# dmMaze/comic-text-detector

Measured on AMD Instinct MI355X. Metric: pages/sec at 1024x1024 bs=32 (end-to-end detector, device-resident pages), higher is better.
Workload: dtype f16

## Files before the change

### comic-text-detector_amd/csrc/kernels_post.hip

```cpp
#include <algorithm>

#include "kernels.h"


namespace {

struct Cand {
  float x1, y1, x2, y2;
  float score;
  int cls;
  int idx;
  int alive;
};

__global__ void nms_filter_kernel(const float* __restrict__ blks, int B, int rows, int no, float conf_thres,
                                  Cand* __restrict__ cands, int* __restrict__ counts) {
  const long long total = (long long)B * rows;
  for (long long i = (long long)blockIdx.x * blockDim.x + threadIdx.x; i < total;
       i += (long long)gridDim.x * blockDim.x) {
    const int b = (int)(i / rows), r = (int)(i % rows);
    const float* x = blks + i * no;
    const float obj = x[4];
    if (!(obj > conf_thres)) continue;
    float best = x[5] * obj;
    int bj = 0;
    for (int j = 1; j < no - 5; ++j) {
      const float c = x[5 + j] * obj;
      if (c > best) { best = c; bj = j; }
    }
    if (!(best > conf_thres)) continue;
    const int pos = atomicAdd(&counts[b], 1);
    Cand c;
    c.x1 = x[0] - x[2] / 2;
    c.y1 = x[1] - x[3] / 2;
    c.x2 = x[0] + x[2] / 2;
    c.y2 = x[1] + x[3] / 2;
    c.score = best;
    c.cls = bj;
    c.idx = r;
    c.alive = 1;
    cands[(size_t)b * rows + pos] = c;
  }
}

struct Best { float s; int idx; int pos; };
constexpr int NMS_THREADS = 256;
constexpr int NMS_REG = 8;

__device__ __forceinline__ bool better(const Best& a, const Best& b) {
  return a.s > b.s || (a.s == b.s && a.idx < b.idx);
}

__device__ __forceinline__ Best block_argmax(Best v, Best* sh) {
  for (int off = 32; off > 0; off >>= 1) {
    Best o;
    o.s = __shfl_down(v.s, off);
    o.idx = __shfl_down(v.idx, off);
    o.pos = __shfl_down(v.pos, off);
    if (better(o, v)) v = o;
  }
  const int w = threadIdx.x >> 6, l = threadIdx.x & 63;
  __syncthreads();
  if (l == 0) sh[w] = v;
  __syncthreads();
  Best r = sh[0];
  for (int i = 1; i < (int)(blockDim.x >> 6); ++i)
    if (better(sh[i], r)) r = sh[i];
  return r;
}

__global__ __launch_bounds__(NMS_THREADS) void nms_greedy_kernel(Cand* __restrict__ cands_all, const int* __restrict__ counts,
                                                          int rows, float iou_thres, int max_det, int max_nms,
                                                          float max_wh, float* __restrict__ dets,
                                                          int* __restrict__ out_counts) {
  __shared__ Best sh[16];
  __shared__ unsigned cnt_sh;
  const int b = blockIdx.x;
  Cand* c = cands_all + (size_t)b * rows;
  const int n = counts[b];
  float* out = dets + (size_t)b * max_det * 6;

  if (n > max_nms) {
    unsigned prefix = 0;
// ... 455 lines not shown
  constexpr int LU = 4;
  for (int pb = p_begin; pb < p_end; pb += 256 * LU) {
    int root[LU], idv[LU];
#pragma unroll
    for (int u = 0; u < LU; ++u) {
      const int p = pb + 256 * u + threadIdx.x;
      root[u] = p < p_end ? labels_all[base + p] : -1;
    }
#pragma unroll
    for (int u = 0; u < LU; ++u) idv[u] = root[u] >= 0 ? ids_all[base + root[u]] : 0;
#pragma unroll
    for (int u = 0; u < LU; ++u) {
      const int p = pb + 256 * u + threadIdx.x;
      if (p < p_end && !(bg_negative && root[u] < 0)) labels_all[base + p] = idv[u];
    }
    if (!stats) continue;
#pragma unroll
    for (int u = 0; u < LU; ++u) {
      const int p0 = pb + 256 * u;
      if (p0 >= p_end) break;
      const int p = p0 + threadIdx.x;
      const bool live = p < p_end;
      const int id = idv[u];
      const int x = live ? p % W : 0, y = live ? p / W : 0;
      const int key = live ? id : -1;
      const int prev = __shfl_up(key, 1);
      const bool head = lane == 0 || prev != key || x == 0;
      const unsigned long long heads = __ballot(head);
      if (head && id > 0 && id <= max_labels) {
        const unsigned long long later = lane == 63 ? 0ull : (heads >> (lane + 1));
        const int len = later ? __ffsll((long long)later) : 64 - lane;
        int slot = -1;
        unsigned hsh = ((unsigned)id * 2654435761u) >> 25;
        for (int probe = 0; probe < 4; ++probe) {
          const int sidx = (hsh + probe) & (LB_SLOTS - 1);
          const int old = atomicCAS(&hkey[sidx], -1, id);
          if (old == -1 || old == id) {
            slot = sidx;
            break;
          }
        }
        int* s = slot >= 0 ? hst + 5 * slot : stats + ((size_t)b * max_labels + (id - 1)) * 5;
        atomicMin(s + 0, x);
        atomicMin(s + 1, y);
        atomicMax(s + 2, x + len - 1);
        atomicMax(s + 3, y);
        atomicAdd(s + 4, len);
      }
    }
  }
  if (stats) {
    __syncthreads();
    for (int sl = threadIdx.x; sl < LB_SLOTS; sl += 256) {
      const int id = hkey[sl];
      if (id <= 0) continue;
      int* s = stats + ((size_t)b * max_labels + (id - 1)) * 5;
      atomicMin(s + 0, hst[5 * sl]);
      atomicMin(s + 1, hst[5 * sl + 1]);
      atomicMax(s + 2, hst[5 * sl + 2]);
      atomicMax(s + 3, hst[5 * sl + 3]);
      atomicAdd(s + 4, hst[5 * sl + 4]);
    }
  }
}
__global__ __launch_bounds__(256) void ccl_label_kernel(int* __restrict__ labels_all, const int* __restrict__ ids_all,
                                                        int B, int H, int W, int chunks, int* __restrict__ stats,
                                                        int max_labels, int bg_negative, int nvb) {
  for (int vb = blockIdx.x; vb < nvb; vb += gridDim.x) {
    ccl_label_body(vb, labels_all, ids_all, B, H, W, chunks, stats, max_labels, bg_negative);
    __syncthreads();
  }
}

__global__ void ccl_stats_final_kernel(int* __restrict__ stats, const int* __restrict__ n_out, int max_labels) {
  const int b = blockIdx.y;
  const int n = min(n_out[b], max_labels);
  for (int l = blockIdx.x * blockDim.x + threadIdx.x; l < n; l += gridDim.x * blockDim.x) {
    int* s = stats + ((size_t)b * max_labels + l) * 5;
    s[2] = s[2] - s[0] + 1;
    s[3] = s[3] - s[1] + 1;
  }
}

__device__ __forceinline__ void ccl2_local_body(int vb, const uint8_t* __restrict__ img, int* __restrict__ parent_all,
                                                         int H, int W, int tiles_x, int tiles_y, int thresh) {
  __shared__ int lp[CT * CT];
  __shared__ unsigned mrow[2][CT];
  int bid = vb;
  const int tx = bid % tiles_x;
  bid /= tiles_x;
  const int ty = bid % tiles_y;
  const int b = bid / tiles_y;
  const size_t base = (size_t)b * H * W;
  const int x0 = tx * CT, y0 = ty * CT;
  const int lane = threadIdx.x & 63;
  const int lx = threadIdx.x & 31;
  int pix[CT * CT / 256];
#pragma unroll
  for (int k = 0; k < CT * CT / 256; ++k) {
    const int gx = x0 + lx, gy = y0 + ((threadIdx.x + 256 * k) >> 5);
    pix[k] = img[base + (gx < W && gy < H ? (size_t)gy * W + gx : (size_t)0)];
  }
#pragma unroll
  for (int k = 0; k < CT * CT / 256; ++k) {
    const int li = threadIdx.x + 256 * k;
    const int ly = li >> 5;
    const int gx = x0 + lx, gy = y0 + ly;
    const bool valid = gx < W && gy < H;
    const bool fg = valid && pix[k] > thresh;
    const unsigned long long balf = __ballot(fg), balv = __ballot(valid);
    const unsigned mf = (unsigned)(lane < 32 ? balf : balf >> 32);
    const unsigned mv = (unsigned)(lane < 32 ? balv : balv >> 32);
    const unsigned mb = mv & ~mf;
    const unsigned mine = fg ? mf : mb;
    const unsigned below = ~mine & ((1u << lx) - 1u);
    const int start = below ? 32 - __clz(below) : 0;
    lp[li] = valid ? (ly << 5) + start : -1;
    if (lx == 0) mrow[0][ly] = mf, mrow[1][ly] = mb;
  }
  __syncthreads();
#pragma unroll
  for (int k = 0; k < CT * CT / 256; ++k) {
    const int li = threadIdx.x + 256 * k;
    const int ly = li >> 5;
    if (ly == 0) continue;
    const int cls = ((mrow[0][ly] >> lx) & 1u) ? 0 : 1;
    const unsigned m = mrow[cls][ly], ma = mrow[cls][ly - 1];
    if (!((m >> lx) & 1u) || (lx > 0 && ((m >> (lx - 1)) & 1u))) continue;
    const unsigned from = m >> lx;
    const int len = (~from) ? __ffs(~from) - 1 : 32 - lx;
    unsigned run = (len >= 32 ? 0xffffffffu : ((1u << len) - 1u)) << lx;
    if (cls == 0) run |= (run << 1) | (run >> 1);
    unsigned ov = ma & run;
    while (ov) {
      const int bpos = __ffs(ov) - 1;
      const unsigned belowa = ~ma & ((1u << bpos) - 1u);
      const int sa = belowa ? 32 - __clz(belowa) : 0;
      lds_union(lp, li, ((ly - 1) << 5) + sa);
      const unsigned froma = ma >> bpos;
      const int lena = (~froma) ? __ffs(~froma) - 1 : 32 - bpos;
      ov &= ~((lena >= 32 ? 0xffffffffu : ((1u << lena) - 1u)) << bpos);
    }
  }
  __syncthreads();
#pragma unroll
  for (int k = 0; k < CT * CT / 256; ++k) {
    const int li = threadIdx.x + 256 * k;
    const int gx = x0 + lx, gy = y0 + (li >> 5);
    if (gx >= W || gy >= H) continue;
    const int r = lds_find(lp, lp[li]);
    parent_all[base + (size_t)gy * W + gx] = (y0 + (r >> 5)) * W + x0 + (r & 31);
  }
}
__global__ __launch_bounds__(256) void ccl2_local_kernel(const uint8_t* __restrict__ img, int* __restrict__ parent_all,
                                                         int H, int W, int tiles_x, int tiles_y, int thresh, int nvb) {
  for (int vb = blockIdx.x; vb < nvb; vb += gridDim.x) {
    ccl2_local_body(vb, img, parent_all, H, W, tiles_x, tiles_y, thresh);
    __syncthreads();
  }
}

__global__ __launch_bounds__(256) void ccl2_border_h_kernel(int* __restrict__ parent_all, const uint8_t* __restrict__ img_all,
                                                            int thresh, int H, int W) {
  const int x = blockIdx.x * 256 + threadIdx.x;
  const int y = CT * (blockIdx.y + 1);
  if (x >= W || y >= H) return;
  int* parent = parent_all + (size_t)blockIdx.z * H * W;
  const uint8_t* img = img_all + (size_t)blockIdx.z * H * W;
  const int p = y * W + x;
  const bool me = (int)img[p] > thresh;
  auto same = [&](int q) { return ((int)img[q] > thresh) == me; };
  const bool q = x > 0 && same(p - 1);
  const bool up = same(p - W);
  const bool ul = x > 0 && same(p - W - 1);
  if (!me) {
    if (up && !(q && ul)) uf_union(parent, p, p - W);
    return;
  }
  const bool ur = x + 1 < W && same(p - W + 1);
  if (q) {
    if (ur && !up) uf_union(parent, p, p - W + 1);
  } else if (up) {
    uf_union(parent, p, p - W);
  } else {
    if (ul) uf_union(parent, p, p - W - 1);
    if (ur) uf_union(parent, p, p - W + 1);
  }
}

__global__ __launch_bounds__(256) void ccl2_border_v_kernel(int* __restrict__ parent_all, const uint8_t* __restrict__ img_all,
                                                            int thresh, int H, int W) {
  const int y = blockIdx.x * 256 + threadIdx.x;
  const int x = CT * (blockIdx.y + 1);
  if (y >= H || x >= W) return;
  int* parent = parent_all + (size_t)blockIdx.z * H * W;
  const uint8_t* img = img_all + (size_t)blockIdx.z * H * W;
  const int p = y * W + x;
  const bool ua = y > 0, same_tile = (y % CT) != 0;
  const bool fme = (int)img[p] > thresh, fleft = (int)img[p - 1] > thresh;
  const bool fmu = ua && (int)img[p - W] > thresh, flu = ua && (int)img[p - W - 1] > thresh;
  {
    const bool me = !fme, left = !fleft, mu = ua && !fmu, lu = ua && !flu;
    if (me && left && !(same_tile && mu && lu)) uf_union(parent, p, p - 1);
  }
  {
    const bool me = fme, left = fleft, mu = fmu, lu = flu;
    if (!me && !left) return;
    if (!same_tile) {
      if (me && left) uf_union(parent, p, p - 1);
      if (me && lu) uf_union(parent, p, p - W - 1);
      if (left && mu) uf_union(parent, p - 1, p - W);
      return;
    }
    if (me && left && !(mu && lu)) uf_union(parent, p, p - 1);
    if (me && lu && !left && !mu) uf_union(parent, p, p - W - 1);
    if (left && mu && !me && !lu) uf_union(parent, p - 1, p - W);
  }
}

__device__ __forceinline__ void ccl2_flatten_count_body(int vb, int* __restrict__ parent_all, const uint8_t* __restrict__ img_all,
                                                                 int thresh, int hw, int nchunks, int* __restrict__ chunk_cnt,
                                                                 unsigned long long* __restrict__ rootmask) {
  __shared__ int sh[4];
  const int b = vb / nchunks, ch = vb % nchunks;
  int* parent = parent_all + (size_t)b * hw;
  const uint8_t* img = img_all + (size_t)b * hw;
  const int p0 = ch * RK_CHUNK + threadIdx.x;
  int lf = 0, lb = 0;
  constexpr int FU = 4;
  static_assert(RK_PER_T % FU == 0, "whole batches");
  for (int j0 = 0; j0 < RK_PER_T; j0 += FU) {
    int v[FU], g[FU], px[FU];
#pragma unroll
    for (int j = 0; j < FU; ++j) {
      const int p = p0 + 256 * (j0 + j);
      v[j] = p < hw ? uf_load(parent, p) : -1;
      px[j] = img[min(p, hw - 1)];
    }
#pragma unroll
    for (int j = 0; j < FU; ++j) g[j] = v[j] >= 0 ? uf_load(parent, v[j]) : -1;
#pragma unroll
    for (int j = 0; j < FU; ++j) {
      const int p = p0 + 256 * (j0 + j);
      bool rf = false, rb = false;
      if (v[j] >= 0) {
        const int r = g[j] == v[j] ? v[j] : uf_find(parent, g[j]);
        if (r != v[j]) parent[p] = r;
        if (r == p) {
          if (px[j] > thresh) ++lf, rf = true; else ++lb, rb = true;
        }
      }
      const unsigned long long mf = __ballot(rf), mb = __ballot(rb);
      if ((threadIdx.x & 63) == 0) {
        const size_t wi = (size_t)ch * 64 + 4 * (j0 + j) + (threadIdx.x >> 6);
        rootmask[((size_t)b * 2 + 0) * nchunks * 64 + wi] = mf;
        rootmask[((size_t)b * 2 + 1) * nchunks * 64 + wi] = mb;
      }
    }
  }
  int tf, tb;
  block_exclusive_scan(lf, sh, &tf);
  block_exclusive_scan(lb, sh, &tb);
  if (threadIdx.x == 0) {
    chunk_cnt[((size_t)b * 2 + 0) * nchunks + ch] = tf;
    chunk_cnt[((size_t)b * 2 + 1) * nchunks + ch] = tb;
  }
}
__global__ __launch_bounds__(256) void ccl2_flatten_count_kernel(int* __restrict__ parent_all, const uint8_t* __restrict__ img_all,
                                                                 int thresh, int hw, int nchunks, int* __restrict__ chunk_cnt,
                                                                 unsigned long long* __restrict__ rootmask, int nvb) {
  for (int vb = blockIdx.x; vb < nvb; vb += gridDim.x) {
    ccl2_flatten_count_body(vb, parent_all, img_all, thresh, hw, nchunks, chunk_cnt, rootmask);
    __syncthreads();
  }
}

__global__ __launch_bounds__(256) void ccl2_scan_chunks_kernel(int* __restrict__ chunk_cnt, int nchunks, int* __restrict__ n_f,
                                                               int* __restrict__ n_b) {
  __shared__ int sh[4];
  int* c = chunk_cnt + (size_t)blockIdx.x * nchunks;
  int carry = 0;
  for (int base = 0; base < nchunks; base += 256) {
    const int i = base + threadIdx.x;
    const int v = i < nchunks ? c[i] : 0;
    int total;
    const int excl = block_exclusive_scan(v, sh, &total);
    if (i < nchunks) c[i] = carry + excl;
    carry += total;
    __syncthreads();
  }
  if (threadIdx.x == 0) ((blockIdx.x & 1) ? n_b : n_f)[blockIdx.x >> 1] = carry;
}

__device__ __forceinline__ void ccl2_rank_body(int vb, const unsigned long long* __restrict__ rootmask,
                                                        int hw, int nchunks, const int* __restrict__ chunk_cnt,
                                                        int* __restrict__ ids_all, int* __restrict__ first_f,
                                                        int* __restrict__ first_b, int max_labels) {
  __shared__ int sh[2][4];
  const int b = vb / nchunks, ch = vb % nchunks;
  const int lane = threadIdx.x & 63, w = __builtin_amdgcn_readfirstlane(threadIdx.x >> 6);
  const int base = ch * RK_CHUNK + w * 1024 + lane;
  unsigned long long mf[16], mb[16];
  int cf = 0, cb = 0;
  const unsigned long long* wf = rootmask + ((size_t)b * 2 + 0) * nchunks * 64 + (size_t)ch * 64 + w * 16;
  const unsigned long long* wb = rootmask + ((size_t)b * 2 + 1) * nchunks * 64 + (size_t)ch * 64 + w * 16;
#pragma unroll
  for (int j = 0; j < 16; ++j) {
    mf[j] = wf[j];
    mb[j] = wb[j];
    cf += __popcll(mf[j]);
    cb += __popcll(mb[j]);
  }
  if (lane == 0) sh[0][w] = cf, sh[1][w] = cb;
  __syncthreads();
  int idf = chunk_cnt[((size_t)b * 2 + 0) * nchunks + ch], idb = chunk_cnt[((size_t)b * 2 + 1) * nchunks + ch];
  for (int i = 0; i < w; ++i) idf += sh[0][i], idb += sh[1][i];
  int* ids = ids_all + (size_t)b * hw;
  const unsigned long long below = lane ? (~0ull >> (64 - lane)) : 0ull;
#pragma unroll
  for (int j = 0; j < 16; ++j) {
    const int p = base + 64 * j;
    if ((mf[j] >> lane) & 1ull) {
      const int id = idf + __popcll(mf[j] & below) + 1;
      ids[p] = id;
      if (id <= max_labels) first_f[(size_t)b * max_labels + id - 1] = p;
    } else if ((mb[j] >> lane) & 1ull) {
      const int id = idb + __popcll(mb[j] & below) + 1;
      ids[p] = -id;
      if (id <= max_labels) first_b[(size_t)b * max_labels + id - 1] = p;
    }
    idf += __popcll(mf[j]);
    idb += __popcll(mb[j]);
  }
}
__global__ __launch_bounds__(256) void ccl2_rank_kernel(const unsigned long long* __restrict__ rootmask,
                                                        int hw, int nchunks, const int* __restrict__ chunk_cnt,
                                                        int* __restrict__ ids_all, int* __restrict__ first_f,
                                                        int* __restrict__ first_b, int max_labels, int nvb) {
  for (int vb = blockIdx.x; vb < nvb; vb += gridDim.x) {
    ccl2_rank_body(vb, rootmask, hw, nchunks, chunk_cnt, ids_all, first_f, first_b, max_labels);
    __syncthreads();
  }
}

__device__ __forceinline__ void ccl2_label_body(int vb, int* __restrict__ labels_all, const int* __restrict__ ids_all, int B, int H,
                                                         int W, int chunks, int* __restrict__ st_f, int* __restrict__ st_b,
                                                         int max_labels, uint8_t* __restrict__ seg_live) {
  constexpr int EMPTY = (int)0x80000000;
  __shared__ int hkey[LB_SLOTS];
  __shared__ int hst[LB_SLOTS * 5];
  const int hw = H * W;
  const int b = vb / chunks, ch = vb % chunks;
  const int p_begin = ch * LB_CHUNK, p_end = min(hw, p_begin + LB_CHUNK);
  const size_t base = (size_t)b * hw;
  for (int s = threadIdx.x; s < LB_SLOTS; s += 256) {
    hkey[s] = EMPTY;
    hst[5 * s] = W, hst[5 * s + 1] = H, hst[5 * s + 2] = -1, hst[5 * s + 3] = -1, hst[5 * s + 4] = 0;
  }
  __syncthreads();
  const int lane = threadIdx.x & 63;
  auto row_of = [&](int id) { return (id > 0 ? st_f : st_b) + ((size_t)b * max_labels + ((id > 0 ? id : -id) - 1)) * 5; };
  constexpr int LU = 4;
  for (int pb = p_begin; pb < p_end; pb += 256 * LU) {
    int root[LU], idv[LU];
#pragma unroll
    for (int u = 0; u < LU; ++u) {
      const int p = pb + 256 * u + threadIdx.x;
      root[u] = p < p_end ? labels_all[base + p] : -1;
    }
#pragma unroll
    for (int u = 0; u < LU; ++u) idv[u] = root[u] >= 0 ? ids_all[base + root[u]] : 0;
#pragma unroll
    for (int u = 0; u < LU; ++u) {
      const int p = pb + 256 * u + threadIdx.x;
      if (p < p_end) labels_all[base + p] = idv[u];
    }
#pragma unroll
    for (int u = 0; u < LU; ++u) {
      const int p0 = pb + 256 * u;
      if (p0 >= p_end) break;
      const int p = p0 + threadIdx.x;
      const bool live = p < p_end;
      const int id = idv[u];
      const int x = live ? p % W : 0, y = live ? p / W : 0;
      if (seg_live) {
        const unsigned long long other = __ballot(live && id != -1);
        const int q0 = p0 + ((int)threadIdx.x & ~63);
        if (lane == 0 && q0 < p_end) seg_live[(size_t)b * ((hw + 63) >> 6) + (q0 >> 6)] = other ? 1 : 0;
      }
      const int prev = __shfl_up(id, 1);
      const bool head = lane == 0 || prev != id || x == 0;
      const unsigned long long heads = __ballot(head);
      const int mag = id > 0 ? id : -id;
      if (head && id != 0 && mag <= max_labels) {
        const unsigned long long later = lane == 63 ? 0ull : (heads >> (lane + 1));
        const int len = later ? __ffsll((long long)later) : 64 - lane;
        int slot = -1;
        const unsigned hsh = ((unsigned)id * 2654435761u) >> 25;
        for (int probe = 0; probe < 4; ++probe) {
          const int sidx = (hsh + probe) & (LB_SLOTS - 1);
          const int old = atomicCAS(&hkey[sidx], EMPTY, id);
          if (old == EMPTY || old == id) {
            slot = sidx;
            break;
          }
        }
        int* s = slot >= 0 ? hst + 5 * slot : row_of(id);
        atomicMin(s + 0, x);
        atomicMin(s + 1, y);
        atomicMax(s + 2, x + len - 1);
        atomicMax(s + 3, y);
        atomicAdd(s + 4, len);
      }
    }
  }
  __syncthreads();
  for (int sl = threadIdx.x; sl < LB_SLOTS; sl += 256) {
    const int id = hkey[sl];
    if (id == EMPTY) continue;
    int* s = row_of(id);
    atomicMin(s + 0, hst[5 * sl]);
    atomicMin(s + 1, hst[5 * sl + 1]);
    atomicMax(s + 2, hst[5 * sl + 2]);
    atomicMax(s + 3, hst[5 * sl + 3]);
    atomicAdd(s + 4, hst[5 * sl + 4]);
  }
}
__global__ __launch_bounds__(256) void ccl2_label_kernel(int* __restrict__ labels_all, const int* __restrict__ ids_all, int B, int H,
                                                         int W, int chunks, int* __restrict__ st_f, int* __restrict__ st_b,
                                                         int max_labels, int nvb, uint8_t* __restrict__ seg_live) {
  for (int vb = blockIdx.x; vb < nvb; vb += gridDim.x) {
    ccl2_label_body(vb, labels_all, ids_all, B, H, W, chunks, st_f, st_b, max_labels, seg_live);
    __syncthreads();
  }
}


inline int capped(int nvb) { return std::max(1, std::min(nvb, g_tail_max_blocks)); }

inline int grid_for(long long total, int block = 256) {
  long long g = (total + block - 1) / block;
  if (g > (long long)g_tail_max_blocks) g = g_tail_max_blocks;
  if (g < 1) g = 1;
  return (int)g;
}

template <int CONN>
void launch_border(int* labels, const unsigned* colmask, int B, int H, int W, hipStream_t st) {
  const int nh = (H - 1) / CT, nv = (W - 1) / CT;
  if (nh > 0) hipLaunchKernelGGL((ccl_border_h_kernel<CONN>), dim3((W + 255) / 256, nh, B), dim3(256), 0, st, labels, H, W);
  if (nv > 0)
    hipLaunchKernelGGL((ccl_border_v_kernel<CONN>), dim3((H + 255) / 256, nv, B), dim3(256), 0, st, labels, colmask, H, W,
                       (W + CT - 1) / CT, (H + CT - 1) / CT);
}

}

size_t nms_workspace_bytes(int B, int rows) { return (size_t)B * rows * sizeof(Cand) + (size_t)B * sizeof(int) + 256; }

void launch_nms(const float* blks, int B, int rows, int no, float conf, float iou, int max_det, int max_nms,
                float max_wh, float* dets, int* counts, void* ws, hipStream_t st) {
  int* cnt = (int*)ws;
  Cand* cands = (Cand*)((char*)ws + ((size_t)B * sizeof(int) + 255) / 256 * 256);
  (void)hipMemsetAsync(cnt, 0, (size_t)B * sizeof(int), st);
  (void)hipMemsetAsync(dets, 0, (size_t)B * max_det * 6 * sizeof(float), st);
  hipLaunchKernelGGL(nms_filter_kernel, dim3(grid_for((long long)B * rows)), dim3(256), 0, st, blks, B, rows, no, conf,
                     cands, cnt);
  hipLaunchKernelGGL(nms_greedy_kernel, dim3(B), dim3(NMS_THREADS), 0, st, cands, cnt, rows, iou, max_det, max_nms, max_wh,
                     dets, counts);
}

size_t ccl_workspace_bytes(int B, int H, int W) {
  const size_t hw = (size_t)H * W;
  const size_t nchunks = (hw + RK_CHUNK - 1) / RK_CHUNK;
  const size_t tiles_max = hw / (CT * CT) + (hw + 1) / CT + 2;
  return (size_t)B * hw * sizeof(int) + 2 * (size_t)B * nchunks * sizeof(int) + 2 * (size_t)B * nchunks * 64 * 8 +
         (size_t)B * tiles_max * 2 * sizeof(unsigned) + 1280;
}

void launch_ccl(const uint8_t* img, int B, int H, int W, int thresh, int conn, int* labels, int* n_out, int* stats,
                int max_labels, void* ws, hipStream_t st, int invert, int* first, int bg_negative) {
  const int hw = H * W;
  const long long total = (long long)B * hw;
  const int nchunks = (hw + RK_CHUNK - 1) / RK_CHUNK;
  int* ids = (int*)ws;
  int* chunk_cnt = (int*)((char*)ws + ((size_t)total * sizeof(int) + 255) / 256 * 256);
  unsigned long long* rootmask = (unsigned long long*)((char*)chunk_cnt + ((size_t)B * nchunks * sizeof(int) + 255) / 256 * 256);
  unsigned* colmask = (unsigned*)((char*)rootmask + ((size_t)B * nchunks * 64 * 8 + 255) / 256 * 256);
  const int tiles_x = (W + CT - 1) / CT, tiles_y = (H + CT - 1) / CT;
  if (conn == 8) {
    hipLaunchKernelGGL((ccl_local_kernel<8>), dim3(capped(B * tiles_x * tiles_y)), dim3(256), 0, st, img, labels, colmask, H, W,
                       tiles_x, tiles_y, thresh, invert, B * tiles_x * tiles_y);
    launch_border<8>(labels, colmask, B, H, W, st);
  } else {
    hipLaunchKernelGGL((ccl_local_kernel<4>), dim3(capped(B * tiles_x * tiles_y)), dim3(256), 0, st, img, labels, colmask, H, W,
                       tiles_x, tiles_y, thresh, invert, B * tiles_x * tiles_y);
    launch_border<4>(labels, colmask, B, H, W, st);
  }
  hipLaunchKernelGGL(ccl_flatten_count_kernel, dim3(capped(B * nchunks)), dim3(256), 0, st, labels, hw, nchunks, chunk_cnt, rootmask,
                     B * nchunks);
  hipLaunchKernelGGL(ccl_scan_chunks_kernel, dim3(B), dim3(256), 0, st, chunk_cnt, nchunks, n_out);
  hipLaunchKernelGGL(ccl_rank_kernel, dim3(capped(B * nchunks)), dim3(256), 0, st, rootmask, hw, nchunks, chunk_cnt, ids, first,
                     max_labels, B * nchunks);
  const int sgrid = std::max(1, std::min(64, (max_labels + 255) / 256));
  if (stats) hipLaunchKernelGGL(ccl_stats_init_kernel, dim3(sgrid, B), dim3(256), 0, st, stats, n_out, max_labels, H, W);
  const int lchunks = (hw + LB_CHUNK - 1) / LB_CHUNK;
  hipLaunchKernelGGL(ccl_label_kernel, dim3(capped(B * lchunks)), dim3(256), 0, st, labels, ids, B, H, W, lchunks, stats, max_labels,
                     bg_negative, B * lchunks);
  if (stats) hipLaunchKernelGGL(ccl_stats_final_kernel, dim3(sgrid, B), dim3(256), 0, st, stats, n_out, max_labels);
}

void launch_ccl_dual(const uint8_t* img, int B, int H, int W, int thresh, int* labels, int* n_f, int* n_b, int* st_f,
                     int* st_b, int* first_f, int* first_b, int max_labels, void* ws, hipStream_t st, uint8_t* seg_live) {
  const int hw = H * W;
  const long long total = (long long)B * hw;
  const int nchunks = (hw + RK_CHUNK - 1) / RK_CHUNK;
  int* ids = (int*)ws;
  int* chunk_cnt = (int*)((char*)ws + ((size_t)total * sizeof(int) + 255) / 256 * 256);
  unsigned long long* rootmask = (unsigned long long*)((char*)chunk_cnt + (2 * (size_t)B * nchunks * sizeof(int) + 255) / 256 * 256);
  const int tiles_x = (W + CT - 1) / CT, tiles_y = (H + CT - 1) / CT;
  hipLaunchKernelGGL(ccl2_local_kernel, dim3(capped(B * tiles_x * tiles_y)), dim3(256), 0, st, img, labels, H, W, tiles_x, tiles_y,
                     thresh, B * tiles_x * tiles_y);
  const int nh = (H - 1) / CT, nv = (W - 1) / CT;
  if (nh > 0) hipLaunchKernelGGL(ccl2_border_h_kernel, dim3((W + 255) / 256, nh, B), dim3(256), 0, st, labels, img, thresh, H, W);
  if (nv > 0) hipLaunchKernelGGL(ccl2_border_v_kernel, dim3((H + 255) / 256, nv, B), dim3(256), 0, st, labels, img, thresh, H, W);
  hipLaunchKernelGGL(ccl2_flatten_count_kernel, dim3(capped(B * nchunks)), dim3(256), 0, st, labels, img, thresh, hw, nchunks, chunk_cnt,
                     rootmask, B * nchunks);
  hipLaunchKernelGGL(ccl2_scan_chunks_kernel, dim3(2 * B), dim3(256), 0, st, chunk_cnt, nchunks, n_f, n_b);
  hipLaunchKernelGGL(ccl2_rank_kernel, dim3(capped(B * nchunks)), dim3(256), 0, st, rootmask, hw, nchunks, chunk_cnt, ids,
                     first_f, first_b, max_labels, B * nchunks);
  const int sgrid = std::max(1, std::min(64, (max_labels + 255) / 256));
  hipLaunchKernelGGL(ccl_stats_init_kernel, dim3(sgrid, B), dim3(256), 0, st, st_f, n_f, max_labels, H, W);
  hipLaunchKernelGGL(ccl_stats_init_kernel, dim3(sgrid, B), dim3(256), 0, st, st_b, n_b, max_labels, H, W);
  const int lchunks = (hw + LB_CHUNK - 1) / LB_CHUNK;
  hipLaunchKernelGGL(ccl2_label_kernel, dim3(capped(B * lchunks)), dim3(256), 0, st, labels, ids, B, H, W, lchunks, st_f, st_b,
                     max_labels, B * lchunks, seg_live);
  hipLaunchKernelGGL(ccl_stats_final_kernel, dim3(sgrid, B), dim3(256), 0, st, st_f, n_f, max_labels);
  hipLaunchKernelGGL(ccl_stats_final_kernel, dim3(sgrid, B), dim3(256), 0, st, st_b, n_b, max_labels);
}
```

Measured before the change: 3306.

## Rewrite dual connected-component labeling to operate on bit-packed horizontal runs

Replaces the per-pixel tile union-find CCL with a run-based scheme. The thresholded image is packed into bit words with run-start masks, run ids come from a prefix scan, and union-find runs over runs within 32-row bands in LDS, with a separate border pass between bands. The label kernel then resolves each pixel's label through the run tables, and first-pixel recording moves into the label pass. The aim is fewer union-find nodes and less per-pixel global traffic in exchange for more kernels and more workspace, with a global-memory fallback when a band holds more runs than fit in LDS.

```diff
diff --git a/comic-text-detector_amd/csrc/kernels_post.hip b/comic-text-detector_amd/csrc/kernels_post.hip
--- a/comic-text-detector_amd/csrc/kernels_post.hip
+++ b/comic-text-detector_amd/csrc/kernels_post.hip
@@ -1,4 +1,5 @@
 #include <algorithm>
+#include <cstdint>
 
 #include "kernels.h"
 
@@ -620,149 +621,249 @@
   }
 }
 
-__device__ __forceinline__ void ccl2_local_body(int vb, const uint8_t* __restrict__ img, int* __restrict__ parent_all,
-                                                         int H, int W, int tiles_x, int tiles_y, int thresh) {
-  __shared__ int lp[CT * CT];
-  __shared__ unsigned mrow[2][CT];
-  int bid = vb;
-  const int tx = bid % tiles_x;
-  bid /= tiles_x;
-  const int ty = bid % tiles_y;
-  const int b = bid / tiles_y;
-  const size_t base = (size_t)b * H * W;
-  const int x0 = tx * CT, y0 = ty * CT;
-  const int lane = threadIdx.x & 63;
-  const int lx = threadIdx.x & 31;
-  int pix[CT * CT / 256];
-#pragma unroll
-  for (int k = 0; k < CT * CT / 256; ++k) {
-    const int gx = x0 + lx, gy = y0 + ((threadIdx.x + 256 * k) >> 5);
-    pix[k] = img[base + (gx < W && gy < H ? (size_t)gy * W + gx : (size_t)0)];
-  }
-#pragma unroll
-  for (int k = 0; k < CT * CT / 256; ++k) {
-    const int li = threadIdx.x + 256 * k;
-    const int ly = li >> 5;
-    const int gx = x0 + lx, gy = y0 + ly;
-    const bool valid = gx < W && gy < H;
-    const bool fg = valid && pix[k] > thresh;
-    const unsigned long long balf = __ballot(fg), balv = __ballot(valid);
-    const unsigned mf = (unsigned)(lane < 32 ? balf : balf >> 32);
-    const unsigned mv = (unsigned)(lane < 32 ? balv : balv >> 32);
-    const unsigned mb = mv & ~mf;
-    const unsigned mine = fg ? mf : mb;
-    const unsigned below = ~mine & ((1u << lx) - 1u);
-    const int start = below ? 32 - __clz(below) : 0;
-    lp[li] = valid ? (ly << 5) + start : -1;
-    if (lx == 0) mrow[0][ly] = mf, mrow[1][ly] = mb;
-  }
-  __syncthreads();
-#pragma unroll
-  for (int k = 0; k < CT * CT / 256; ++k) {
-    const int li = threadIdx.x + 256 * k;
-    const int ly = li >> 5;
-    if (ly == 0) continue;
-    const int cls = ((mrow[0][ly] >> lx) & 1u) ? 0 : 1;
-    const unsigned m = mrow[cls][ly], ma = mrow[cls][ly - 1];
-    if (!((m >> lx) & 1u) || (lx > 0 && ((m >> (lx - 1)) & 1u))) continue;
-    const unsigned from = m >> lx;
-    const int len = (~from) ? __ffs(~from) - 1 : 32 - lx;
-    unsigned run = (len >= 32 ? 0xffffffffu : ((1u << len) - 1u)) << lx;
-    if (cls == 0) run |= (run << 1) | (run >> 1);
-    unsigned ov = ma & run;
-    while (ov) {
-      const int bpos = __ffs(ov) - 1;
-      const unsigned belowa = ~ma & ((1u << bpos) - 1u);
-      const int sa = belowa ? 32 - __clz(belowa) : 0;
-      lds_union(lp, li, ((ly - 1) << 5) + sa);
-      const unsigned froma = ma >> bpos;
-      const int lena = (~froma) ? __ffs(~froma) - 1 : 32 - bpos;
-      ov &= ~((lena >= 32 ? 0xffffffffu : ((1u << lena) - 1u)) << bpos);
-    }
-  }
-  __syncthreads();
-#pragma unroll
-  for (int k = 0; k < CT * CT / 256; ++k) {
-    const int li = threadIdx.x + 256 * k;
-    const int gx = x0 + lx, gy = y0 + (li >> 5);
-    if (gx >= W || gy >= H) continue;
-    const int r = lds_find(lp, lp[li]);
-    parent_all[base + (size_t)gy * W + gx] = (y0 + (r >> 5)) * W + x0 + (r & 31);
-  }
-}
-__global__ __launch_bounds__(256) void ccl2_local_kernel(const uint8_t* __restrict__ img, int* __restrict__ parent_all,
-                                                         int H, int W, int tiles_x, int tiles_y, int thresh, int nvb) {
+struct RunTables {
+  const unsigned* starts;
+  const unsigned* base;
+  const int* rlabel;
+  int wp;
+};
+constexpr int RB_ROWS = 32;
+constexpr int RB_THREADS = 1024;
+constexpr int RB_CAP = 8192;
+
+constexpr int PK_U = 4;
+constexpr int PK_SEG = 32 * PK_U;
+__device__ __forceinline__ void ccl2_pack_body(int vb, const uint8_t* __restrict__ img, unsigned* __restrict__ bits_all,
+                                                        unsigned* __restrict__ starts_all, int* __restrict__ segsum, int nseg, int H,
+                                                        int W, int wp, int thresh, int aligned4) {
+  __shared__ int segc;
+  const int nw = H * wp;
+  const size_t hw = (size_t)H * W;
+  const int b = vb / nseg, seg = vb - b * nseg;
+  if (threadIdx.x == 0) segc = 0;
+  __syncthreads();
+  unsigned px[PK_U];
+  int prev[PK_U], xs[PK_U], ws[PK_U];
+#pragma unroll
+  for (int u = 0; u < PK_U; ++u) {
+    const int g = (int)threadIdx.x;
+    const int rem = seg * PK_SEG + u * 32 + (g >> 3);
+    const bool valid = rem < nw;
+    const int y = valid ? rem / wp : 0, wx = valid ? rem - y * wp : 0;
+    const int x = wx * 32 + 4 * (g & 7);
+    const uint8_t* row = img + (size_t)b * hw + (size_t)y * W;
+    unsigned v = 0;
+    if (valid && x < W) {
+      if (aligned4) {
+        v = *reinterpret_cast<const unsigned*>(row + x);
+      } else {
+#pragma unroll
+        for (int k = 0; k < 4; ++k)
+          if (x + k < W) v |= (unsigned)row[x + k] << (8 * k);
+      }
+    }
+    px[u] = v;
+    prev[u] = (valid && ((int)g & 7) == 0 && wx > 0) ? (int)row[x - 1] : -1;
+    xs[u] = x;
+    ws[u] = valid ? rem : -1;
+  }
+  unsigned* bits = bits_all + (size_t)b * nw;
+  unsigned* starts = starts_all + (size_t)b * nw;
+  int nstart = 0;
+#pragma unroll
+  for (int u = 0; u < PK_U; ++u) {
+    const int x = xs[u];
+    unsigned nib = 0;
+#pragma unroll
+    for (int k = 0; k < 4; ++k)
+      if (x + k < W && (int)((px[u] >> (8 * k)) & 255u) > thresh) nib |= 1u << k;
+    unsigned v = nib << (4 * (threadIdx.x & 7));
+    v |= __shfl_xor(v, 1);
+    v |= __shfl_xor(v, 2);
+    v |= __shfl_xor(v, 4);
+    if ((threadIdx.x & 7) == 0 && ws[u] >= 0) {
+      const int nbit = min(32, W - x);
+      const unsigned vmask = nbit >= 32 ? 0xffffffffu : ((1u << nbit) - 1u);
+      const unsigned pb = prev[u] >= 0 ? (prev[u] > thresh ? 1u : 0u) : (~v & 1u);
+      const unsigned s = (v ^ ((v << 1) | pb)) & vmask;
+      bits[ws[u]] = v;
+      starts[ws[u]] = s;
+      nstart += __popc(s);
+    }
+  }
+  if (nstart) atomicAdd(&segc, nstart);
+  __syncthreads();
+  if (threadIdx.x == 0) segsum[vb] = segc;
+}
+__global__ __launch_bounds__(256) void ccl2_pack_kernel(const uint8_t* __restrict__ img, unsigned* __restrict__ bits_all,
+                                                        unsigned* __restrict__ starts_all, int* __restrict__ segsum, int nseg, int H,
+                                                        int W, int wp, int thresh, int aligned4, int nvb) {
   for (int vb = blockIdx.x; vb < nvb; vb += gridDim.x) {
-    ccl2_local_body(vb, img, parent_all, H, W, tiles_x, tiles_y, thresh);
-    __syncthreads();
-  }
-}
-
-__global__ __launch_bounds__(256) void ccl2_border_h_kernel(int* __restrict__ parent_all, const uint8_t* __restrict__ img_all,
-                                                            int thresh, int H, int W) {
-  const int x = blockIdx.x * 256 + threadIdx.x;
-  const int y = CT * (blockIdx.y + 1);
-  if (x >= W || y >= H) return;
-  int* parent = parent_all + (size_t)blockIdx.z * H * W;
-  const uint8_t* img = img_all + (size_t)blockIdx.z * H * W;
-  const int p = y * W + x;
-  const bool me = (int)img[p] > thresh;
-  auto same = [&](int q) { return ((int)img[q] > thresh) == me; };
-  const bool q = x > 0 && same(p - 1);
-  const bool up = same(p - W);
-  const bool ul = x > 0 && same(p - W - 1);
-  if (!me) {
-    if (up && !(q && ul)) uf_union(parent, p, p - W);
+    ccl2_pack_body(vb, img, bits_all, starts_all, segsum, nseg, H, W, wp, thresh, aligned4);
+    __syncthreads();
+  }
+}
+
+constexpr int SC_TILE = 4096;
+static_assert(SC_TILE % PK_SEG == 0 && SC_TILE == 256 * 16, "whole segments; 16 words per thread");
+__device__ __forceinline__ void ccl2_run_scan_body(int vb, const unsigned* __restrict__ starts_all, const int* __restrict__ segsum,
+                                                            unsigned* __restrict__ base_all, int* __restrict__ rcount, int nw, int nseg,
+                                                            int ntiles) {
+  __shared__ int sh[4];
+  const int b = vb / ntiles, tile = vb - b * ntiles;
+  const unsigned* starts = starts_all + (size_t)b * nw;
+  unsigned* base = base_all + (size_t)b * nw;
+  const int i0 = tile * SC_TILE + 16 * (int)threadIdx.x;
+  unsigned sv[16];
+#pragma unroll
+  for (int k = 0; k < 16; ++k) sv[k] = i0 + k < nw ? starts[i0 + k] : 0u;
+  int before = 0;
+  for (int i = threadIdx.x; i < tile * (SC_TILE / PK_SEG); i += 256) before += segsum[(size_t)b * nseg + i];
+  int mine = 0;
+#pragma unroll
+  for (int k = 0; k < 16; ++k) mine += __popc(sv[k]);
+  int prefix, total;
+  block_exclusive_scan(before, sh, &prefix);
+  int e = prefix + block_exclusive_scan(mine, sh, &total);
+#pragma unroll
+  for (int k = 0; k < 16; ++k) {
+    if (i0 + k < nw) base[i0 + k] = (unsigned)e;
+    e += __popc(sv[k]);
+  }
+  if (tile == ntiles - 1 && threadIdx.x == 0) rcount[b] = prefix + total;
+}
+__global__ __launch_bounds__(256) void ccl2_run_scan_kernel(const unsigned* __restrict__ starts_all, const int* __restrict__ segsum,
+                                                            unsigned* __restrict__ base_all, int* __restrict__ rcount, int nw, int nseg,
+                                                            int ntiles, int nvb) {
+  for (int vb = blockIdx.x; vb < nvb; vb += gridDim.x) {
+    ccl2_run_scan_body(vb, starts_all, segsum, base_all, rcount, nw, nseg, ntiles);
+    __syncthreads();
+  }
+}
+
+template <class U>
+__device__ __forceinline__ void ccl2_word_unions(const unsigned* __restrict__ bits, const unsigned* __restrict__ starts,
+                                                          const unsigned* __restrict__ base, int y, int wx, int wp, int W, U&& unite) {
+  const int w = y * wp + wx, wa = w - wp;
+  const bool hl = wx > 0, hr = wx + 1 < wp;
+  const unsigned c = bits[w], sc = starts[w], a = bits[wa], sa = starts[wa];
+  const int bc = (int)base[w], ba = (int)base[wa];
+  const unsigned al = hl ? bits[wa - 1] : 0u, sal = hl ? starts[wa - 1] : 0u;
+  const int bal = hl ? (int)base[wa - 1] : 0;
+  const unsigned ar = hr ? bits[wa + 1] : 0u, sar = hr ? starts[wa + 1] : 0u;
+  const int bar = hr ? (int)base[wa + 1] : 0;
+  const int nbit = min(32, W - 32 * wx);
+  const unsigned vmask = nbit >= 32 ? 0xffffffffu : ((1u << nbit) - 1u);
+#pragma unroll
+  for (int cls = 0; cls < 2; ++cls) {
+    const unsigned m = (cls ? c : ~c) & vmask, ma = (cls ? a : ~a) & vmask;
+    unsigned rest = m;
+    while (rest) {
+      const int lo = __ffs(rest) - 1;
+      const unsigned from = m >> lo;
+      const int len = (~from) ? __ffs(~from) - 1 : 32 - lo;
+      const unsigned g = (len >= 32 ? 0xffffffffu : ((1u << len) - 1u)) << lo;
+      rest &= ~g;
+      const int me = bc + __popc(sc & ((2u << lo) - 1u)) - 1;
+      const bool cont = lo == 0 && !(sc & 1u);
+      unsigned reach = g;
+      if (cls) reach |= (g << 1) | (g >> 1);
+      unsigned ov = ma & reach;
+      while (ov) {
+        const int bpos = __ffs(ov) - 1;
+        if (!(cont && bpos == 0 && !(sa & 1u))) unite(me, ba + __popc(sa & ((2u << bpos) - 1u)) - 1);
+        const unsigned froma = ma >> bpos;
+        const int lena = (~froma) ? __ffs(~froma) - 1 : 32 - bpos;
+        ov &= ~((lena >= 32 ? 0xffffffffu : ((1u << lena) - 1u)) << bpos);
+      }
+      if (cls) {
+        if (lo == 0 && (al >> 31)) unite(me, bal + __popc(sal) - 1);
+        if (lo + len == 32 && (ar & 1u)) unite(me, bar + (int)(sar & 1u) - 1);
+      }
+    }
+  }
+}
+
+__device__ __forceinline__ void ccl2_band_body(int vb, const unsigned* __restrict__ bits_all, const unsigned* __restrict__ starts_all,
+                                                        const unsigned* __restrict__ base_all, const int* __restrict__ rcount,
+                                                        int* __restrict__ rparent_all, uint8_t* __restrict__ rcls_all, int H, int W,
+                                                        int wp, int nbands) {
+  __shared__ int lp[RB_CAP];
+  const int b = vb / nbands, k = vb % nbands;
+  const int y0 = k * RB_ROWS, y1 = min(H, y0 + RB_ROWS);
+  const size_t nw = (size_t)H * wp, hw = (size_t)H * W;
+  const unsigned* bits = bits_all + b * nw;
+  const unsigned* starts = starts_all + b * nw;
+  const unsigned* base = base_all + b * nw;
+  int* rparent = rparent_all + b * hw;
+  uint8_t* rcls = rcls_all + b * hw;
+  const int gbase = (int)base[y0 * wp];
+  const int n = (y1 < H ? (int)base[y1 * wp] : rcount[b]) - gbase;
+  const bool in_lds = n <= RB_CAP;
+  if (in_lds) {
+    for (int i = threadIdx.x; i < n; i += RB_THREADS) lp[i] = i;
+  } else {
+    for (int i = threadIdx.x; i < n; i += RB_THREADS) rparent[gbase + i] = gbase + i;
+    __threadfence();
+  }
+  __syncthreads();
+  for (int wi = y0 * wp + threadIdx.x; wi < y1 * wp; wi += RB_THREADS) {
+    const int y = wi / wp, wx = wi - y * wp;
+    unsigned s = starts[wi];
+    const unsigned c = bits[wi];
+    int id = (int)base[wi];
+    while (s) {
+      const int pos = __ffs(s) - 1;
+      s &= s - 1u;
+      rcls[id++] = (uint8_t)((c >> pos) & 1u);
+    }
+    if (y == y0) continue;
+    if (in_lds)
+      ccl2_word_unions(bits, starts, base, y, wx, wp, W, [&](int p, int q) { lds_union(lp, p - gbase, q - gbase); });
+    else
+      ccl2_word_unions(bits, starts, base, y, wx, wp, W, [&](int p, int q) { uf_union(rparent, p, q); });
+  }
+  __syncthreads();
+  if (in_lds)
+    for (int i = threadIdx.x; i < n; i += RB_THREADS) rparent[gbase + i] = gbase + lds_find(lp, i);
+}
+__global__ __launch_bounds__(RB_THREADS) void ccl2_band_kernel(const unsigned* __restrict__ bits_all, const unsigned* __restrict__ starts_all,
+                                                        const unsigned* __restrict__ base_all, const int* __restrict__ rcount,
+                                                        int* __restrict__ rparent_all, uint8_t* __restrict__ rcls_all, int H, int W,
+                                                        int wp, int nbands, int nvb) {
+  for (int vb = blockIdx.x; vb < nvb; vb += gridDim.x) {
+    ccl2_band_body(vb, bits_all, starts_all, base_all, rcount, rparent_all, rcls_all, H, W, wp, nbands);
+    __syncthreads();
+  }
+}
+
+__global__ __launch_bounds__(256) void ccl2_band_border_kernel(const unsigned* __restrict__ bits_all,
+                                                               const unsigned* __restrict__ starts_all,
+                                                               const unsigned* __restrict__ base_all, int* __restrict__ rparent_all,
+                                                               int B, int H, int W, int wp, int nbord) {
+  int t = blockIdx.x * 256 + threadIdx.x;
+  if (t >= B * nbord * wp) return;
+  const int wx = t % wp;
+  t /= wp;
+  const int k = t % nbord, b = t / nbord;
+  const size_t nw = (size_t)H * wp;
+  int* rparent = rparent_all + (size_t)b * H * W;
+  ccl2_word_unions(bits_all + b * nw, starts_all + b * nw, base_all + b * nw, RB_ROWS * (k + 1), wx, wp, W,
+                   [&](int p, int q) { uf_union(rparent, p, q); });
+}
+
+__device__ __forceinline__ void ccl2_flatten_count_body(int vb, int* __restrict__ parent_all, const uint8_t* __restrict__ rcls_all,
+                                                                 const int* __restrict__ rcount, int B, int hw, int nchunks,
+                                                                 int* __restrict__ chunk_cnt, unsigned long long* __restrict__ rootmask) {
+  __shared__ int sh[4];
+  const int b = vb % B, ch = vb / B;
+  const int R = rcount[b];
+  if (ch * RK_CHUNK >= R) {
+    if (threadIdx.x == 0) chunk_cnt[((size_t)b * 2 + 0) * nchunks + ch] = 0, chunk_cnt[((size_t)b * 2 + 1) * nchunks + ch] = 0;
     return;
   }
-  const bool ur = x + 1 < W && same(p - W + 1);
-  if (q) {
-    if (ur && !up) uf_union(parent, p, p - W + 1);
-  } else if (up) {
-    uf_union(parent, p, p - W);
-  } else {
-    if (ul) uf_union(parent, p, p - W - 1);
-    if (ur) uf_union(parent, p, p - W + 1);
-  }
-}
-
-__global__ __launch_bounds__(256) void ccl2_border_v_kernel(int* __restrict__ parent_all, const uint8_t* __restrict__ img_all,
-                                                            int thresh, int H, int W) {
-  const int y = blockIdx.x * 256 + threadIdx.x;
-  const int x = CT * (blockIdx.y + 1);
-  if (y >= H || x >= W) return;
-  int* parent = parent_all + (size_t)blockIdx.z * H * W;
-  const uint8_t* img = img_all + (size_t)blockIdx.z * H * W;
-  const int p = y * W + x;
-  const bool ua = y > 0, same_tile = (y % CT) != 0;
-  const bool fme = (int)img[p] > thresh, fleft = (int)img[p - 1] > thresh;
-  const bool fmu = ua && (int)img[p - W] > thresh, flu = ua && (int)img[p - W - 1] > thresh;
-  {
-    const bool me = !fme, left = !fleft, mu = ua && !fmu, lu = ua && !flu;
-    if (me && left && !(same_tile && mu && lu)) uf_union(parent, p, p - 1);
-  }
-  {
-    const bool me = fme, left = fleft, mu = fmu, lu = flu;
-    if (!me && !left) return;
-    if (!same_tile) {
-      if (me && left) uf_union(parent, p, p - 1);
-      if (me && lu) uf_union(parent, p, p - W - 1);
-      if (left && mu) uf_union(parent, p - 1, p - W);
-      return;
-    }
-    if (me && left && !(mu && lu)) uf_union(parent, p, p - 1);
-    if (me && lu && !left && !mu) uf_union(parent, p, p - W - 1);
-    if (left && mu && !me && !lu) uf_union(parent, p - 1, p - W);
-  }
-}
-
-__device__ __forceinline__ void ccl2_flatten_count_body(int vb, int* __restrict__ parent_all, const uint8_t* __restrict__ img_all,
-                                                                 int thresh, int hw, int nchunks, int* __restrict__ chunk_cnt,
-                                                                 unsigned long long* __restrict__ rootmask) {
-  __shared__ int sh[4];
-  const int b = vb / nchunks, ch = vb % nchunks;
   int* parent = parent_all + (size_t)b * hw;
-  const uint8_t* img = img_all + (size_t)b * hw;
+  const uint8_t* rcls = rcls_all + (size_t)b * hw;
   const int p0 = ch * RK_CHUNK + threadIdx.x;
   int lf = 0, lb = 0;
   constexpr int FU = 4;
@@ -772,8 +873,8 @@
 #pragma unroll
     for (int j = 0; j < FU; ++j) {
       const int p = p0 + 256 * (j0 + j);
-      v[j] = p < hw ? uf_load(parent, p) : -1;
-      px[j] = img[min(p, hw - 1)];
+      v[j] = p < R ? uf_load(parent, p) : -1;
+      px[j] = rcls[min(p, R - 1)];
     }
 #pragma unroll
     for (int j = 0; j < FU; ++j) g[j] = v[j] >= 0 ? uf_load(parent, v[j]) : -1;
@@ -784,8 +885,9 @@
       if (v[j] >= 0) {
         const int r = g[j] == v[j] ? v[j] : uf_find(parent, g[j]);
         if (r != v[j]) parent[p] = r;
+        if (g[j] != v[j] && r != g[j]) parent[v[j]] = r;
         if (r == p) {
-          if (px[j] > thresh) ++lf, rf = true; else ++lb, rb = true;
+          if (px[j]) ++lf, rf = true; else ++lb, rb = true;
         }
       }
       const unsigned long long mf = __ballot(rf), mb = __ballot(rb);
@@ -804,11 +906,12 @@
     chunk_cnt[((size_t)b * 2 + 1) * nchunks + ch] = tb;
   }
 }
-__global__ __launch_bounds__(256) void ccl2_flatten_count_kernel(int* __restrict__ parent_all, const uint8_t* __restrict__ img_all,
-                                                                 int thresh, int hw, int nchunks, int* __restrict__ chunk_cnt,
-                                                                 unsigned long long* __restrict__ rootmask, int nvb) {
+__global__ __launch_bounds__(256) void ccl2_flatten_count_kernel(int* __restrict__ parent_all, const uint8_t* __restrict__ rcls_all,
+                                                                 const int* __restrict__ rcount, int B, int hw, int nchunks,
+                                                                 int* __restrict__ chunk_cnt, unsigned long long* __restrict__ rootmask,
+                                                                 int nvb) {
   for (int vb = blockIdx.x; vb < nvb; vb += gridDim.x) {
-    ccl2_flatten_count_body(vb, parent_all, img_all, thresh, hw, nchunks, chunk_cnt, rootmask);
+    ccl2_flatten_count_body(vb, parent_all, rcls_all, rcount, B, hw, nchunks, chunk_cnt, rootmask);
     __syncthreads();
   }
 }
@@ -830,12 +933,12 @@
   if (threadIdx.x == 0) ((blockIdx.x & 1) ? n_b : n_f)[blockIdx.x >> 1] = carry;
 }
 
-__device__ __forceinline__ void ccl2_rank_body(int vb, const unsigned long long* __restrict__ rootmask,
-                                                        int hw, int nchunks, const int* __restrict__ chunk_cnt,
-                                                        int* __restrict__ ids_all, int* __restrict__ first_f,
-                                                        int* __restrict__ first_b, int max_labels) {
+__device__ __forceinline__ void ccl2_rank_body(int vb, const unsigned long long* __restrict__ rootmask, const int* __restrict__ rcount,
+                                                        int B, int hw, int nchunks, const int* __restrict__ chunk_cnt,
+                                                        int* __restrict__ ids_all) {
   __shared__ int sh[2][4];
-  const int b = vb / nchunks, ch = vb % nchunks;
+  const int b = vb % B, ch = vb / B;
+  if (ch * RK_CHUNK >= rcount[b]) return;
   const int lane = threadIdx.x & 63, w = __builtin_amdgcn_readfirstlane(threadIdx.x >> 6);
   const int base = ch * RK_CHUNK + w * 1024 + lane;
   unsigned long long mf[16], mb[16];
@@ -860,30 +963,57 @@
     const int p = base + 64 * j;
     if ((mf[j] >> lane) & 1ull) {
       const int id = idf + __popcll(mf[j] & below) + 1;
-      ids[p] = id;
-      if (id <= max_labels) first_f[(size_t)b * max_labels + id - 1] = p;
+      ids[p] = 2 * id + 1;
     } else if ((mb[j] >> lane) & 1ull) {
       const int id = idb + __popcll(mb[j] & below) + 1;
-      ids[p] = -id;
-      if (id <= max_labels) first_b[(size_t)b * max_labels + id - 1] = p;
+      ids[p] = -2 * id + 1;
     }
     idf += __popcll(mf[j]);
     idb += __popcll(mb[j]);
   }
 }
-__global__ __launch_bounds__(256) void ccl2_rank_kernel(const unsigned long long* __restrict__ rootmask,
-                                                        int hw, int nchunks, const int* __restrict__ chunk_cnt,
-                                                        int* __restrict__ ids_all, int* __restrict__ first_f,
-                                                        int* __restrict__ first_b, int max_labels, int nvb) {
+__global__ __launch_bounds__(256) void ccl2_rank_kernel(const unsigned long long* __restrict__ rootmask, const int* __restrict__ rcount,
+                                                        int B, int hw, int nchunks, const int* __restrict__ chunk_cnt,
+                                                        int* __restrict__ ids_all, int nvb) {
   for (int vb = blockIdx.x; vb < nvb; vb += gridDim.x) {
-    ccl2_rank_body(vb, rootmask, hw, nchunks, chunk_cnt, ids_all, first_f, first_b, max_labels);
-    __syncthreads();
-  }
-}
-
-__device__ __forceinline__ void ccl2_label_body(int vb, int* __restrict__ labels_all, const int* __restrict__ ids_all, int B, int H,
+    ccl2_rank_body(vb, rootmask, rcount, B, hw, nchunks, chunk_cnt, ids_all);
+    __syncthreads();
+  }
+}
+
+__global__ __launch_bounds__(256) void ccl2_spread_kernel(const int* __restrict__ rparent_all, const int* __restrict__ rcount, int B,
+                                                          int hw, int nchunks, int* __restrict__ rlabel_all, int nvb) {
+  for (int vb = blockIdx.x; vb < nvb; vb += gridDim.x) {
+    const int b = vb % B, ch = vb / B;
+    const int R = rcount[b];
+    const int* rparent = rparent_all + (size_t)b * hw;
+    int* rlabel = rlabel_all + (size_t)b * hw;
+    constexpr int SU = 4;
+    for (int j0 = 0; j0 < RK_PER_T && ch * RK_CHUNK + 256 * j0 < R; j0 += SU) {
+      int par[SU], lab[SU];
+#pragma unroll
+      for (int j = 0; j < SU; ++j) {
+        const int r = ch * RK_CHUNK + 256 * (j0 + j) + threadIdx.x;
+        par[j] = r < R ? rparent[r] : -1;
+      }
+#pragma unroll
+      for (int j = 0; j < SU; ++j) {
+        const int r = ch * RK_CHUNK + 256 * (j0 + j) + threadIdx.x;
+        lab[j] = (par[j] >= 0 && par[j] != r) ? rlabel[par[j]] : 0;
+      }
+#pragma unroll
+      for (int j = 0; j < SU; ++j) {
+        const int r = ch * RK_CHUNK + 256 * (j0 + j) + threadIdx.x;
+        if (par[j] >= 0 && par[j] != r) rlabel[r] = lab[j] & ~1;
+      }
+    }
+  }
+}
+
+__device__ __forceinline__ void ccl2_label_body(int vb, int* __restrict__ labels_all, const RunTables t, int B, int H,
                                                          int W, int chunks, int* __restrict__ st_f, int* __restrict__ st_b,
-                                                         int max_labels, uint8_t* __restrict__ seg_live) {
+                                                         int* __restrict__ first_f, int* __restrict__ first_b, int max_labels,
+                                                         uint8_t* __restrict__ seg_live) {
   constexpr int EMPTY = (int)0x80000000;
   __shared__ int hkey[LB_SLOTS];
   __shared__ int hst[LB_SLOTS * 5];
@@ -891,6 +1021,9 @@
   const int b = vb / chunks, ch = vb % chunks;
   const int p_begin = ch * LB_CHUNK, p_end = min(hw, p_begin + LB_CHUNK);
   const size_t base = (size_t)b * hw;
+  const unsigned* starts = t.starts + (size_t)b * H * t.wp;
+  const unsigned* wbase = t.base + (size_t)b * H * t.wp;
+  const int* rlabel = t.rlabel + base;
   for (int s = threadIdx.x; s < LB_SLOTS; s += 256) {
     hkey[s] = EMPTY;
     hst[5 * s] = W, hst[5 * s + 1] = H, hst[5 * s + 2] = -1, hst[5 * s + 3] = -1, hst[5 * s + 4] = 0;
@@ -898,16 +1031,31 @@
   __syncthreads();
   const int lane = threadIdx.x & 63;
   auto row_of = [&](int id) { return (id > 0 ? st_f : st_b) + ((size_t)b * max_labels + ((id > 0 ? id : -id) - 1)) * 5; };
-  constexpr int LU = 4;
+  constexpr int LU = 8;
+  static_assert(LB_CHUNK % (256 * LU) == 0, "whole batches");
   for (int pb = p_begin; pb < p_end; pb += 256 * LU) {
-    int root[LU], idv[LU];
+    unsigned sw[LU];
+    int run[LU], idv[LU];
 #pragma unroll
     for (int u = 0; u < LU; ++u) {
       const int p = pb + 256 * u + threadIdx.x;
-      root[u] = p < p_end ? labels_all[base + p] : -1;
-    }
-#pragma unroll
-    for (int u = 0; u < LU; ++u) idv[u] = root[u] >= 0 ? ids_all[base + root[u]] : 0;
+      const int y = p / W, w = y * t.wp + ((p - y * W) >> 5);
+      sw[u] = p < p_end ? starts[w] : 0u;
+      run[u] = p < p_end ? (int)wbase[w] : 0;
+    }
+#pragma unroll
+    for (int u = 0; u < LU; ++u) {
+      const int p = pb + 256 * u + threadIdx.x;
+      const int bit = (p % W) & 31;
+      run[u] += __popc(sw[u] & ((2u << bit) - 1u)) - 1;
+      idv[u] = p < p_end ? rlabel[run[u]] : 0;
+      sw[u] = (sw[u] >> bit) & 1u;
+    }
+#pragma unroll
+    for (int u = 0; u < LU; ++u) {
+      sw[u] &= (unsigned)idv[u];
+      idv[u] >>= 1;
+    }
 #pragma unroll
     for (int u = 0; u < LU; ++u) {
       const int p = pb + 256 * u + threadIdx.x;
@@ -930,6 +1078,7 @@
       const bool head = lane == 0 || prev != id || x == 0;
       const unsigned long long heads = __ballot(head);
       const int mag = id > 0 ? id : -id;
+      if (sw[u] && mag <= max_labels) (id > 0 ? first_f : first_b)[(size_t)b * max_labels + mag - 1] = p;
       if (head && id != 0 && mag <= max_labels) {
         const unsigned long long later = lane == 63 ? 0ull : (heads >> (lane + 1));
         const int len = later ? __ffsll((long long)later) : 64 - lane;
@@ -964,11 +1113,12 @@
     atomicAdd(s + 4, hst[5 * sl + 4]);
   }
 }
-__global__ __launch_bounds__(256) void ccl2_label_kernel(int* __restrict__ labels_all, const int* __restrict__ ids_all, int B, int H,
+__global__ __launch_bounds__(256) void ccl2_label_kernel(int* __restrict__ labels_all, const RunTables t, int B, int H,
                                                          int W, int chunks, int* __restrict__ st_f, int* __restrict__ st_b,
-                                                         int max_labels, int nvb, uint8_t* __restrict__ seg_live) {
+                                                         int* __restrict__ first_f, int* __restrict__ first_b, int max_labels,
+                                                         int nvb, uint8_t* __restrict__ seg_live) {
   for (int vb = blockIdx.x; vb < nvb; vb += gridDim.x) {
-    ccl2_label_body(vb, labels_all, ids_all, B, H, W, chunks, st_f, st_b, max_labels, seg_live);
+    ccl2_label_body(vb, labels_all, t, B, H, W, chunks, st_f, st_b, first_f, first_b, max_labels, seg_live);
     __syncthreads();
   }
 }
@@ -1012,8 +1162,11 @@
   const size_t hw = (size_t)H * W;
   const size_t nchunks = (hw + RK_CHUNK - 1) / RK_CHUNK;
   const size_t tiles_max = hw / (CT * CT) + (hw + 1) / CT + 2;
+  const size_t nw = (size_t)H * ((W + 31) / 32);
+  const size_t run_tables = (size_t)B * hw + 3 * (size_t)B * nw * sizeof(unsigned) + (size_t)B * sizeof(int) +
+                            (size_t)B * (nw / 128 + 1) * sizeof(int);
   return (size_t)B * hw * sizeof(int) + 2 * (size_t)B * nchunks * sizeof(int) + 2 * (size_t)B * nchunks * 64 * 8 +
-         (size_t)B * tiles_max * 2 * sizeof(unsigned) + 1280;
+         std::max((size_t)B * tiles_max * 2 * sizeof(unsigned), run_tables) + 2560;
 }
 
 void launch_ccl(const uint8_t* img, int B, int H, int W, int thresh, int conn, int* labels, int* n_out, int* stats,
@@ -1053,26 +1206,45 @@
   const int hw = H * W;
   const long long total = (long long)B * hw;
   const int nchunks = (hw + RK_CHUNK - 1) / RK_CHUNK;
-  int* ids = (int*)ws;
-  int* chunk_cnt = (int*)((char*)ws + ((size_t)total * sizeof(int) + 255) / 256 * 256);
-  unsigned long long* rootmask = (unsigned long long*)((char*)chunk_cnt + (2 * (size_t)B * nchunks * sizeof(int) + 255) / 256 * 256);
-  const int tiles_x = (W + CT - 1) / CT, tiles_y = (H + CT - 1) / CT;
-  hipLaunchKernelGGL(ccl2_local_kernel, dim3(capped(B * tiles_x * tiles_y)), dim3(256), 0, st, img, labels, H, W, tiles_x, tiles_y,
-                     thresh, B * tiles_x * tiles_y);
-  const int nh = (H - 1) / CT, nv = (W - 1) / CT;
-  if (nh > 0) hipLaunchKernelGGL(ccl2_border_h_kernel, dim3((W + 255) / 256, nh, B), dim3(256), 0, st, labels, img, thresh, H, W);
-  if (nv > 0) hipLaunchKernelGGL(ccl2_border_v_kernel, dim3((H + 255) / 256, nv, B), dim3(256), 0, st, labels, img, thresh, H, W);
-  hipLaunchKernelGGL(ccl2_flatten_count_kernel, dim3(capped(B * nchunks)), dim3(256), 0, st, labels, img, thresh, hw, nchunks, chunk_cnt,
-                     rootmask, B * nchunks);
+  const int wp = (W + 31) / 32, nw = H * wp;
+  auto after = [](void* p, size_t bytes) { return (void*)((char*)p + (bytes + 255) / 256 * 256); };
+  int* rlabel = (int*)ws;
+  int* chunk_cnt = (int*)after(rlabel, (size_t)total * sizeof(int));
+  unsigned long long* rootmask = (unsigned long long*)after(chunk_cnt, 2 * (size_t)B * nchunks * sizeof(int));
+  uint8_t* rcls = (uint8_t*)after(rootmask, 2 * (size_t)B * nchunks * 64 * 8);
+  unsigned* bits = (unsigned*)after(rcls, (size_t)total);
+  unsigned* starts = (unsigned*)after(bits, (size_t)B * nw * sizeof(unsigned));
+  unsigned* base = (unsigned*)after(starts, (size_t)B * nw * sizeof(unsigned));
+  int* rcount = (int*)after(base, (size_t)B * nw * sizeof(unsigned));
+  const int nseg = (nw + PK_SEG - 1) / PK_SEG, ntiles = (nw + SC_TILE - 1) / SC_TILE;
+  int* segsum = (int*)after(rcount, (size_t)B * sizeof(int));
+  int* rparent = labels;
+  const int aligned4 = (W % 4 == 0 && ((uintptr_t)img & 3) == 0) ? 1 : 0;
+  hipLaunchKernelGGL(ccl2_pack_kernel, dim3(capped(B * nseg)), dim3(256), 0, st, img, bits, starts, segsum, nseg, H, W, wp, thresh,
+                     aligned4, B * nseg);
+  hipLaunchKernelGGL(ccl2_run_scan_kernel, dim3(capped(B * ntiles)), dim3(256), 0, st, starts, segsum, base, rcount, nw, nseg, ntiles,
+                     B * ntiles);
+  const int nbands = (H + RB_ROWS - 1) / RB_ROWS;
+  const int band_grid = std::max(1, std::min(B * nbands, g_tail_max_blocks / (RB_THREADS / 256)));
+  hipLaunchKernelGGL(ccl2_band_kernel, dim3(band_grid), dim3(RB_THREADS), 0, st, bits, starts, base, rcount, rparent, rcls, H, W, wp,
+                     nbands, B * nbands);
+  if (nbands > 1)
+    hipLaunchKernelGGL(ccl2_band_border_kernel, dim3((B * (nbands - 1) * wp + 255) / 256), dim3(256), 0, st, bits, starts, base,
+                       rparent, B, H, W, wp, nbands - 1);
+  hipLaunchKernelGGL(ccl2_flatten_count_kernel, dim3(capped(B * nchunks)), dim3(256), 0, st, rparent, rcls, rcount, B, hw, nchunks,
+                     chunk_cnt, rootmask, B * nchunks);
   hipLaunchKernelGGL(ccl2_scan_chunks_kernel, dim3(2 * B), dim3(256), 0, st, chunk_cnt, nchunks, n_f, n_b);
-  hipLaunchKernelGGL(ccl2_rank_kernel, dim3(capped(B * nchunks)), dim3(256), 0, st, rootmask, hw, nchunks, chunk_cnt, ids,
-                     first_f, first_b, max_labels, B * nchunks);
+  hipLaunchKernelGGL(ccl2_rank_kernel, dim3(capped(B * nchunks)), dim3(256), 0, st, rootmask, rcount, B, hw, nchunks, chunk_cnt, rlabel,
+                     B * nchunks);
+  hipLaunchKernelGGL(ccl2_spread_kernel, dim3(capped(B * nchunks)), dim3(256), 0, st, rparent, rcount, B, hw, nchunks, rlabel,
+                     B * nchunks);
   const int sgrid = std::max(1, std::min(64, (max_labels + 255) / 256));
   hipLaunchKernelGGL(ccl_stats_init_kernel, dim3(sgrid, B), dim3(256), 0, st, st_f, n_f, max_labels, H, W);
   hipLaunchKernelGGL(ccl_stats_init_kernel, dim3(sgrid, B), dim3(256), 0, st, st_b, n_b, max_labels, H, W);
   const int lchunks = (hw + LB_CHUNK - 1) / LB_CHUNK;
-  hipLaunchKernelGGL(ccl2_label_kernel, dim3(capped(B * lchunks)), dim3(256), 0, st, labels, ids, B, H, W, lchunks, st_f, st_b,
-                     max_labels, B * lchunks, seg_live);
+  const RunTables t{starts, base, rlabel, wp};
+  hipLaunchKernelGGL(ccl2_label_kernel, dim3(capped(B * lchunks)), dim3(256), 0, st, labels, t, B, H, W, lchunks, st_f, st_b, first_f,
+                     first_b, max_labels, B * lchunks, seg_live);
   hipLaunchKernelGGL(ccl_stats_final_kernel, dim3(sgrid, B), dim3(256), 0, st, st_f, n_f, max_labels);
   hipLaunchKernelGGL(ccl_stats_final_kernel, dim3(sgrid, B), dim3(256), 0, st, st_b, n_b, max_labels);
 }
```

After: 3373, median of 6. +2.0%, better.
